# youmi-zym/TemporalStereo

Hardware: AMD Instinct MI355X
Metric: stereo pairs/sec, FlyingThings3D 540x960 D=192 (aggregation hot path) (higher is better)
Workload: dtype f32

## Files before the change

### temporalstereo_amd/csrc/conv_x6p.hip

```cpp
#include "conv_common.hpp"
#include "conv_x6p.hpp"

namespace {

typedef float f32x16 __attribute__((ext_vector_type(16)));
typedef __attribute__((address_space(3))) void* lds_ptr_t;

constexpr int XP_NC = 16;
constexpr int XP_WROWS = 3 * 9 * 2;
constexpr int XP_WBUF = XP_WROWS * 32;
constexpr int XP_GSLOTS = 10;
constexpr int XP_MAXC = 512;

__device__ __forceinline__ void phase_barrier() {
  asm volatile("s_waitcnt lgkmcnt(0)\n\ts_barrier" ::: "memory");
}

template <int HR>
struct XPG {
  static constexpr int in_rows = HR + 2, QPR = 10, LCOLS = 40, NPIX = in_rows * LCOLS;
  static constexpr int SLOTS = in_rows * QPR;
  static constexpr int NPB = HR / 4;
  static constexpr int HALF_U = 3 * 2 * NPIX;
  static constexpr int NWB = HR == 4 ? 3 : 2;
  static constexpr int SPC = HR == 4 ? 4 : 2;
  static constexpr int NCH = 16 / SPC;
  static constexpr int TILE0 = NWB * XP_WBUF;
  static constexpr size_t lds_bytes = (static_cast<size_t>(TILE0) + 2 * HALF_U) * 16 + (8 * 8 * (NPB * 32 + 4) + 2 * XP_MAXC) * 4;
  static_assert(SPC * SLOTS <= 256, "staging slots");
};

struct XPTile {
  int b, od, co0, ty0, tx0;
  int c0, c1;
  int ks;
};

template <int HR>
__global__ void __launch_bounds__(512, 2)
ig_conv_x6p_kernel(const float* __restrict__ x, const u32x4* __restrict__ w6, const float* __restrict__ scale,
                   const float* __restrict__ shift, float* __restrict__ y, const ts::X6P p) {
  using G = XPG<HR>;
  extern __shared__ __attribute__((aligned(16))) u32x4 ldsp[];
  constexpr int NPIX = G::NPIX, LCOLS = G::LCOLS, NPB = G::NPB;
  const int half = threadIdx.x >> 8, tid = threadIdx.x & 255;
  const int wave = tid >> 6, lane = tid & 63;
  const int px = lane & 31, grp = lane >> 5;
  u32x4* wls = ldsp;
  u32x4* in6 = ldsp + G::TILE0 + half * G::HALF_U;

  const int total = p.total_tiles;
  const int nwg = gridDim.x, g = blockIdx.x;
  int band0, band1, first, step;
  if (p.xcd && nwg % 8 == 0) {
    const int per = (total + 7) / 8, xcd = g & 7;
    band0 = xcd * per; band1 = min(total, band0 + per);
    first = band0 + (g >> 3); step = nwg >> 3;
  } else {
    band0 = 0; band1 = total; first = g; step = nwg;
  }
  const int nchunk = (p.Cin + XP_NC - 1) / XP_NC;
  auto tile_at = [&](int L) {
    XPTile t;
    const int tile = L % p.tiles_pp;
    int r = L / p.tiles_pp;
    const int cog = r % p.co_groups; r /= p.co_groups;
    t.od = r % p.D; r /= p.D;
    t.b = r % p.B; t.ks = r / p.B;
    t.c0 = t.ks * p.kspan; t.c1 = min(nchunk, t.c0 + p.kspan);
    t.co0 = cog * 32;
    t.ty0 = (tile / p.tiles_x) * (2 * HR) + half * HR;
    t.tx0 = (tile % p.tiles_x) * 32;
    return t;
  };
  const unsigned HW = static_cast<unsigned>(p.H) * p.W;
  const unsigned cstride_b = static_cast<unsigned>(p.in_cstride) * 4u;

  constexpr int SPC = G::SPC, NCH = G::NCH;
  const bool stager = tid < SPC * G::SLOTS;
  const int sg = SPC == 2 ? tid / G::SLOTS : tid / (2 * G::SLOTS);
  const int shalf = SPC == 2 ? 0 : (tid & 1);
  const int sslot = SPC == 2 ? tid - sg * G::SLOTS : (tid - sg * 2 * G::SLOTS) >> 1;
  const int srow = sslot / G::QPR, squad = sslot - srow * G::QPR;
  const int lpix = sg * NPIX + srow * LCOLS + 4 * squad;
  const int wsw = (sslot >> 1) & 1;
  const __amdgpu_buffer_rsrc_t wr = ig_rsrc(w6, p.w_bytes);
  const unsigned wchunk_b = static_cast<unsigned>(3 * XP_GSLOTS * 2 * p.coutp) * 16u;

  unsigned long long* trc = (p.trace && g == p.trace_wg && (tid == 0)) ? p.trace + half * 256 : nullptr;
  int ntr = 0;
  auto stamp = [&]() {
    if (trc && ntr < 250) trc[ntr] = __builtin_amdgcn_s_memtime();
    ++ntr;
  };
  stamp();
  unsigned long long* wgt = (p.trace && p.trace_wg == -2 && threadIdx.x == 0 && g < 8000) ? p.trace + 512 + 4 * g : nullptr;
  if (wgt) { wgt[0] = __builtin_amdgcn_s_memtime(); wgt[3] = __builtin_amdgcn_s_memrealtime(); }

  __amdgpu_buffer_rsrc_t xr;
  unsigned goff = kOOB;
  auto aim = [&](const XPTile& t) {
    xr = ig_rsrc(x + static_cast<long long>(t.b) * p.in_bstride, p.in_bytes);
    const int gy = t.ty0 - 1 + srow, gx = t.tx0 - 4 + 4 * squad;
    goff = (stager && gy >= 0 && gy < p.H && gx >= 0 && gx < p.W)
        ? (static_cast<unsigned>(t.od) * HW + static_cast<unsigned>(gy) * p.W + gx) * 4u : kOOB;
  };
  v4f rin[NCH];
  auto fetch = [&](int c) {
#pragma unroll
    for (int e = 0; e < NCH; ++e) {
      const unsigned co = static_cast<unsigned>(min(c * XP_NC + sg * 8 + shalf * 4 + e, p.Cin - 1)) * cstride_b;
      rin[e] = __builtin_bit_cast(v4f, __builtin_amdgcn_raw_buffer_load_b128(xr, (goff == kOOB || (p.dbg & 1)) ? kOOB : goff + co, 0, 0));
    }
  };
  auto dma_weights = [&](int c, int co0, int buf, int share) {
    u32x4* dst = wls + buf * XP_WBUF;
    const unsigned cbase = static_cast<unsigned>(c) * wchunk_b;
    const bool lane_ok = co0 + px < p.coutp && !(p.dbg & 16);
#pragma unroll
    for (int q = 0; q < 7; ++q) {
      const int i = share < 0 ? wave + 4 * q : 2 * (wave + 4 * q) + share;
      if (i < 27 && (share < 0 || q < 4)) {
        const int pt = i / 9, tap = i - pt * 9;
        const unsigned row = static_cast<unsigned>((pt * XP_GSLOTS + tap) * 2 + grp);
        const unsigned off = lane_ok ? (row * p.coutp + co0 + px) * 16u + cbase : kOOB;
        __builtin_amdgcn_raw_ptr_buffer_load_lds(wr, (lds_ptr_t)(dst + i * 64), 16, off, 0, 0, 0);
      }
    }
  };
  auto commit = [&]() {
    if (stager && !(p.dbg & 4)) {
#pragma unroll
      for (int i = 0; i < 4; ++i) {
        unsigned part[3][NCH / 2];
#pragma unroll
        for (int e = 0; e < NCH / 2; ++e) split6(rin[2 * e][i], rin[2 * e + 1][i], part[0][e], part[1][e], part[2][e]);
#pragma unroll
        for (int pt = 0; pt < 3; ++pt) {
          if constexpr (SPC == 2) in6[pt * 2 * NPIX + lpix + (i ^ wsw)] = u32x4{part[pt][0], part[pt][1], part[pt][2], part[pt][3]};
          else reinterpret_cast<u32x2*>(in6 + pt * 2 * NPIX + lpix + (i ^ wsw))[shalf] = u32x2{part[pt][0], part[pt][1]};
        }
      }
    }
  };

  auto swz = [](int P) { return (P & ~3) | ((P & 3) ^ ((P >> 3) & 1)); };
  int rbase[2][3];
#pragma unroll
  for (int rr = 0; rr < 2; ++rr)
#pragma unroll
    for (int kx = 0; kx < 3; ++kx) rbase[rr][kx] = grp * NPIX + swz((wave * NPB + rr) * LCOLS + 3 + kx + px);
  const int aoff = grp * 32 + px;

  constexpr int CH = NPB == 1 ? 2 : 1;
  constexpr int NACC = CH * NPB;
  f32x16 acc[NPB];

  constexpr int EPITCH = NPB * 32 + 4;
  float* scr = reinterpret_cast<float*>(ldsp + G::TILE0 + 2 * G::HALF_U) + (threadIdx.x >> 6) * (8 * EPITCH);
  const float* ss = reinterpret_cast<const float*>(ldsp + G::TILE0 + 2 * G::HALF_U) + 8 * 8 * EPITCH;
  auto epilogue = [&](const XPTile& t) {
    const bool split = p.ksplit > 1;
    const __amdgpu_buffer_rsrc_t yr = split
        ? ig_rsrc(p.partial + (static_cast<size_t>(t.ks) * p.B + t.b) * p.Cout * (static_cast<size_t>(p.D) * HW), p.part_bytes)
        : ig_rsrc(y + static_cast<long long>(t.b) * p.out_bstride, p.out_bytes);
    const unsigned ocs = split ? static_cast<unsigned>(p.D) * HW * 4u : static_cast<unsigned>(p.out_cstride) * 4u;
    const float* ab = (p.addend && !split) ? p.addend + static_cast<size_t>(t.b) * p.add_bstride : nullptr;
    const unsigned obase = static_cast<unsigned>(t.od) * HW;
    if (ab) {
#pragma unroll
      for (int r = 0; r < 16; ++r)
#pragma unroll
        for (int pb = 0; pb < NPB; ++pb) {
          const int oy = t.ty0 + wave * NPB + pb, ox = t.tx0 + px;
          acc[pb][r] += ab[static_cast<size_t>(min(t.co0 + (r & 3) + 8 * (r >> 2) + 4 * grp, p.Cout - 1)) * p.add_cstride +
                           ((oy < p.H && ox < p.W) ? static_cast<unsigned>(oy) * p.W + ox : 0u)];
        }
    }
#pragma unroll
    for (int r = 0; r < 16; ++r) {
      const int cc = min(t.co0 + (r & 3) + 8 * (r >> 2) + 4 * grp, p.coutp - 1);
      const float sc = split ? 1.f : ss[cc], sh = split ? 0.f : ss[XP_MAXC + cc];
#pragma unroll
      for (int pb = 0; pb < NPB; ++pb) acc[pb][r] = acc[pb][r] * sc + sh;
    }
    if (split) {
    } else if (p.act == ACT_SILU) {
#pragma unroll
      for (int r = 0; r < 16; ++r)
#pragma unroll
        for (int pb = 0; pb < NPB; ++pb) acc[pb][r] = silu_fast(acc[pb][r]);
    } else if (p.act == ACT_RELU) {
#pragma unroll
      for (int r = 0; r < 16; ++r)
#pragma unroll
        for (int pb = 0; pb < NPB; ++pb) acc[pb][r] = fmaxf(acc[pb][r], 0.f);
    }
#pragma unroll
    for (int k = 0; k < 4; ++k) {
#pragma unroll
      for (int j = 0; j < 4; ++j)
#pragma unroll
        for (int pb = 0; pb < NPB; ++pb) scr[(j + 4 * grp) * EPITCH + pb * 32 + px] = acc[pb][4 * k + j];
#pragma unroll
      for (int m = 0; m < NPB; ++m) {
        const int i = lane + 64 * m;
        const int c8 = i / (8 * NPB), q = i % (8 * NPB);
        const v4f val = *reinterpret_cast<const v4f*>(scr + c8 * EPITCH + q * 4);
        const int oy = t.ty0 + wave * NPB + (q >> 3), ox = t.tx0 + (q & 7) * 4;
        const int co = t.co0 + 8 * k + c8;
        const unsigned off = (oy < p.H && ox < p.W && co < p.Cout && !(p.dbg & 8))
            ? (obase + static_cast<unsigned>(oy) * p.W + ox) * 4u + static_cast<unsigned>(co) * ocs : kOOB;
        __builtin_amdgcn_raw_buffer_store_b128(__builtin_bit_cast(u32x4, val), yr, off, 0, 0);
      }
    }
  };

  if (first >= band1) return;
  {
    float* ssw = reinterpret_cast<float*>(ldsp + G::TILE0 + 2 * G::HALF_U) + 8 * 8 * EPITCH;
    for (int i = threadIdx.x; i < p.coutp; i += 512) {
      ssw[i] = scale ? scale[i] : 1.f;
      ssw[XP_MAXC + i] = shift ? shift[i] : 0.f;
    }
  }
  XPTile cur = tile_at(first);
  aim(cur);
  fetch(cur.c0);
  constexpr int NWB = G::NWB;
  if (NWB == 3) dma_weights(cur.c0, cur.co0, 0, half);
  else if (half == 1) dma_weights(cur.c0, cur.co0, 0, -1);
  if (half == 1) {
    asm volatile("s_waitcnt vmcnt(0)" ::: "memory");
    phase_barrier();
  }
  stamp();
  int wcur = 0, wnext = 1;
  for (int L = first; L < band1; L += step) {
    const bool more = L + step < band1;
    const XPTile nxt = more ? tile_at(L + step) : cur;
#pragma unroll
    for (int pb = 0; pb < NPB; ++pb)
#pragma unroll
      for (int r = 0; r < 16; ++r) acc[pb][r] = 0.f;
    for (int c = cur.c0; c < cur.c1; ++c, wcur = wnext, wnext = (wnext + 1 == NWB ? 0 : wnext + 1)) {
      const bool last = c + 1 == cur.c1;
      asm volatile("s_waitcnt vmcnt(0)" ::: "memory");
      stamp();
      if ((NWB == 3 || half == 1) && (!last || more))
        dma_weights(last ? nxt.c0 : c + 1, last ? nxt.co0 : cur.co0, wnext, NWB == 3 ? half : -1);
      commit();
      asm volatile("s_waitcnt lgkmcnt(0)" ::: "memory");
      stamp();
      phase_barrier();
      stamp();
      if (!last) fetch(c + 1);
      else if (more) { aim(nxt); fetch(nxt.c0); }
      const u32x4* wb = wls + wcur * XP_WBUF;
      f32x16 part[NACC];
#pragma unroll
      for (int a = 0; a < NACC; ++a)
#pragma unroll
        for (int r = 0; r < 16; ++r) part[a][r] = 0.f;
      bf16x8 af[2][3], bf[2][3][NPB];
      auto load_frag = [&](int tap, int buf) {
        constexpr int OA[3] = {0, 2, 1}, OB[3] = {2, 0, 1};
#pragma unroll
        for (int k = 0; k < 3; ++k) {
          af[buf][OA[k]] = __builtin_bit_cast(bf16x8, wb[(OA[k] * 9 + tap) * 64 + aoff]);
#pragma unroll
          for (int pb = 0; pb < NPB; ++pb) bf[buf][OB[k]][pb] = __builtin_bit_cast(bf16x8, in6[OB[k] * 2 * NPIX + rbase[(pb + tap / 3) & 1][tap % 3] + ((pb + tap / 3) >> 1) * 80]);
        }
      };
      if (!(p.dbg & 2)) {
        load_frag(0, 0);
        __builtin_amdgcn_sched_group_barrier(0x100, 3 + 3 * NPB, 0);
#pragma unroll
        for (int tap = 0; tap < 9; ++tap) {
          if (tap + 1 < 9) load_frag(tap + 1, (tap + 1) & 1);
          constexpr int PA[6] = {0, 2, 1, 0, 1, 0}, PB[6] = {2, 0, 1, 1, 0, 0};
#pragma unroll
          for (int t = 0; t < 6; ++t)
#pragma unroll
            for (int pb = 0; pb < NPB; ++pb) {
              const int a = pb * CH + (t % CH);
              part[a] = __builtin_amdgcn_mfma_f32_32x32x16_bf16(af[tap & 1][PA[t]], bf[tap & 1][PB[t]][pb], part[a], 0, 0, 0);
            }
          if (tap + 1 < 9) {
#pragma unroll
            for (int k = 0; k < 3 + 3 * NPB; ++k) {
              __builtin_amdgcn_sched_group_barrier(0x008, 1, 0);
              __builtin_amdgcn_sched_group_barrier(0x100, 1, 0);
            }
            if constexpr (6 * NPB > 3 + 3 * NPB) __builtin_amdgcn_sched_group_barrier(0x008, 6 * NPB - (3 + 3 * NPB), 0);
          } else {
            __builtin_amdgcn_sched_group_barrier(0x008, 6 * NPB, 0);
          }
        }
      }
#pragma unroll
      for (int pb = 0; pb < NPB; ++pb)
#pragma unroll
        for (int r = 0; r < 16; ++r) {
          float v = part[pb * CH][r];
#pragma unroll
          for (int k = 1; k < CH; ++k) v += part[pb * CH + k][r];
          acc[pb][r] += v;
        }
      if (trc) asm volatile("s_nop 0" :: "v"(acc[0][0]), "v"(acc[NPB - 1][15]));
      stamp();
      if (NWB == 3 || half == 1) asm volatile("s_waitcnt vmcnt(%0)" :: "n"(NCH) : "memory");
      phase_barrier();
      stamp();
    }
    epilogue(cur);
    stamp();
    cur = nxt;
  }
  if (wgt) { asm volatile("s_waitcnt vmcnt(0)" ::: "memory"); wgt[1] = __builtin_amdgcn_s_memtime(); wgt[2] = __builtin_amdgcn_s_memrealtime(); }
  if (half == 0) phase_barrier();
}

template <int HR>
int launch_x6p(const float* x, const void* w6, const float* scale, const float* shift, float* y, const ts::X6P& p, int nwg, hipStream_t st) {
  constexpr size_t lds = XPG<HR>::lds_bytes;
  static_assert(lds <= 160 * 1024, "ig_conv_x6p_kernel: LDS");
  auto kern = &ig_conv_x6p_kernel<HR>;
  static const int attr = hipFuncSetAttribute(reinterpret_cast<const void*>(kern), hipFuncAttributeMaxDynamicSharedMemorySize, static_cast<int>(lds));
  (void)attr;
  hipLaunchKernelGGL(kern, dim3(nwg), dim3(512), lds, st, x, static_cast<const u32x4*>(w6), scale, shift, y, p);
  return ts::launched("ig_conv_x6p_kernel");
}

}

namespace ts {

static unsigned long long* trace_buf = nullptr;
constexpr size_t kTraceBytes = 4096 + 8000 * 32;

static long long tiles_of(const X6P& p, int hr) {
  return static_cast<long long>((p.H + 2 * hr - 1) / (2 * hr)) * ((p.W + 31) / 32) * p.D * p.B * ((p.Cout + 31) / 32) * (p.ksplit > 1 ? p.ksplit : 1);
}

int x6p_rows(const X6P& p) {
  static const long long forced = env_ll("TS_X6P_HR", 0);
  if (forced == 4 || forced == 8) return static_cast<int>(forced);
  const long long r8 = (tiles_of(p, 8) + kNumCU - 1) / kNumCU, r4 = (tiles_of(p, 4) + kNumCU - 1) / kNumCU;
  return 100 * r8 <= 58 * r4 ? 8 : 4;
}

long long x6p_grid(const X6P& p) { return tiles_of(p, 4); }

int x6p_launch(const float* x, const void* w6, const float* scale, const float* shift, float* y, X6P p, void* stream) {
  const int hr = x6p_rows(p);
  static const long long dbg = env_ll("TS_X6P_DBG", 0);
  p.dbg = static_cast<int>(dbg);
  static const long long trace_wg = env_ll("TS_X6P_TRACE", -1);
  if (trace_wg != -1 && !trace_buf) { (void)hipMalloc(reinterpret_cast<void**>(&trace_buf), kTraceBytes); (void)hipMemset(trace_buf, 0, kTraceBytes); }
  p.trace = trace_buf; p.trace_wg = static_cast<int>(trace_wg);
  p.tiles_x = (p.W + 31) / 32;
  p.co_groups = (p.Cout + 31) / 32;
  p.tiles_pp = ((p.H + 2 * hr - 1) / (2 * hr)) * p.tiles_x;
  if (p.ksplit < 1) p.ksplit = 1;
  const long long total = static_cast<long long>(p.tiles_pp) * p.co_groups * p.D * p.B * p.ksplit;
  if (total > 0x3fffffff) return fail(TS_ERR_UNSUPPORTED, "conv3d_hw_x6: too many tiles");
  p.total_tiles = static_cast<int>(total);
  static const long long max_wgs0 = env_ll("TS_X6P_WGS", 208);
  static const long long splitk_all = env_ll("TS_X6P_SPLITK_ALL", 1);
  const long long max_wgs = (splitk_all && p.ksplit > 1 && total <= 256) ? 256 : max_wgs0;
  int nwg = static_cast<int>(total < max_wgs ? total : max_wgs);
  {
    const long long rounds = (total + nwg - 1) / nwg;
    const long long even = (total + rounds - 1) / rounds;
    nwg = static_cast<int>(((even + 7) / 8 * 8 <= nwg) ? (even + 7) / 8 * 8 : even);
  }
  hipStream_t st = as_stream(stream);
  return hr == 8 ? launch_x6p<8>(x, w6, scale, shift, y, p, nwg, st) : launch_x6p<4>(x, w6, scale, shift, y, p, nwg, st);
}

}

extern "C" int ts_x6p_trace_read(unsigned long long* host) {
  if (!ts::trace_buf) return -1;
  (void)hipDeviceSynchronize();
  return static_cast<int>(hipMemcpy(host, ts::trace_buf, ts::kTraceBytes, hipMemcpyDeviceToHost));
}
```

### temporalstereo_amd/csrc/conv_x6s.hip

```cpp
#include "conv_common.hpp"

namespace {

enum { XS_S2 = 0, XS_T3 = 1, XS_T4 = 2 };

template <int MODE, int TR = 8>
struct XG {
  static constexpr bool T = MODE != XS_S2;
  static constexpr int in_rows = T ? TR + 2 : 9;
  static constexpr int QPR = T ? 10 : 18;
  static constexpr int LCOLS = 4 * QPR;
  static constexpr int NPIX = in_rows * LCOLS, NPIXP = NPIX + 1;
  static constexpr int SLOTS = in_rows * QPR;
  static constexpr int NSLOT = T ? 16 : 12;
  static constexpr int NU = T ? 4 : 3;
  static constexpr int NPB = T ? TR / 2 : 2;
  static constexpr int EPI = T ? TR * 64 + 4 : 132;
};
constexpr int kEpiS2 = 132;

inline int slot_tap(int mode, int s) {
  if (mode == XS_S2) return s < 9 ? s : -1;
  const int ks = mode == XS_T4 ? 4 : 3;
  const int cls = s >> 2, a = (s >> 1) & 1, b = s & 1, pa = cls >> 1, pb = cls & 1;
  auto k = [&](int par, int opt) { return par ? (opt ? 0 : 2) : (opt ? (ks == 4 ? 3 : -1) : 1); };
  const int ky = k(pa, a), kx = k(pb, b);
  return (ky < 0 || kx < 0) ? -1 : ky * ks + kx;
}

struct SlotMap { int tap[16]; };

__global__ void __launch_bounds__(256)
weight_split6_g8_kernel(const float* __restrict__ w_t, u32x4* __restrict__ w6, int Cin, int ntaps, int wpad, int coutp, int nchunk,
                        int nslot, const SlotMap m) {
  const int n = nchunk * nslot * coutp;
  for (int i = blockIdx.x * blockDim.x + threadIdx.x; i < n; i += gridDim.x * blockDim.x) {
    const int co = i % coutp;
    const int r = i / coutp;
    const int slot = r % nslot, chunk = r / nslot;
    const int tap = m.tap[slot];
    float v[8];
#pragma unroll
    for (int e = 0; e < 8; ++e) {
      const int ci = chunk * 8 + e;
      v[e] = (tap >= 0 && ci < Cin && co < wpad) ? w_t[(static_cast<size_t>(ci) * ntaps + tap) * wpad + co] : 0.f;
    }
    unsigned part[3][4];
#pragma unroll
    for (int e = 0; e < 4; ++e) split6(v[2 * e], v[2 * e + 1], part[0][e], part[1][e], part[2][e]);
#pragma unroll
    for (int pt = 0; pt < 3; ++pt)
      w6[((static_cast<size_t>(chunk) * 3 + pt) * nslot + slot) * coutp + co] = u32x4{part[pt][0], part[pt][1], part[pt][2], part[pt][3]};
  }
}

template <int MODE, int CB, int TR = 8>
__global__ void __launch_bounds__(256, TR == 4 ? 3 : 2)
ig_conv_x6s_kernel(const float* __restrict__ x, const u32x4* __restrict__ w6, const float* __restrict__ scale,
                   const float* __restrict__ shift, float* __restrict__ y, const IG p) {
  extern __shared__ __attribute__((aligned(16))) u32x4 lds6[];
  using G = XG<MODE, TR>;
  constexpr bool T = G::T;
  static_assert(!T || CB == 1, "transposed forms: 16 output channels per workgroup (four classes of accumulators)");
  constexpr int LCOLS = G::LCOLS, NPIXP = G::NPIXP, NSLOT = G::NSLOT, NU = G::NU, NPB = G::NPB, SLOTS = G::SLOTS;
  constexpr int COB = CB * 16;
  constexpr int WV = 3 * NSLOT * COB, RWN = (WV + 255) / 256;
  constexpr int NCH = T ? 4 : 8;
  u32x4* in6 = lds6;
  u32x4* w6s = lds6 + 3 * NPIXP;

  const int wave = threadIdx.x >> 6, lane = threadIdx.x & 63;
  const int j = lane & 15, kq = lane >> 4;
  unsigned lin = blockIdx.x + gridDim.x * (blockIdx.y + gridDim.y * blockIdx.z);
  {
    const unsigned total = gridDim.x * gridDim.y * gridDim.z, per = total / 8;
    if (p.xcd && lin < per * 8) lin = (lin % 8) * per + lin / 8;
  }
  const int tile = lin % gridDim.x;
  const int od = (lin / gridDim.x) % gridDim.y;
  const int bz = lin / (gridDim.x * gridDim.y);
  const int cog = bz % p.co_groups, b = bz / p.co_groups;
  const int co0 = cog * COB;
  const int ty0 = (tile / p.tiles_x) * (T ? TR : 4), tx0 = (tile % p.tiles_x) * 32;
  const int row0 = T ? ty0 - 1 : 2 * ty0 - 1, col0 = T ? tx0 - 4 : 2 * tx0 - 4;
  const unsigned HW = static_cast<unsigned>(p.H) * p.W;
  const unsigned cstride_b = static_cast<unsigned>(p.in_cstride) * 4u;

  const int half = T ? static_cast<int>(threadIdx.x >> 7) : 0;
  const int sslot = T ? static_cast<int>(threadIdx.x & 127) : static_cast<int>(threadIdx.x);
  const bool stager = sslot < SLOTS;
  const int srow = sslot / G::QPR, squad = sslot - srow * G::QPR;
  unsigned goff = kOOB;
  {
    const int gy = row0 + srow, gx = col0 + 4 * squad;
    if (stager && gy >= 0 && gy < p.H && gx >= 0 && gx < p.W)
      goff = (static_cast<unsigned>(od) * HW + static_cast<unsigned>(gy) * p.W + gx) * 4u;
  }
  const int lpix = srow * LCOLS + 4 * squad;

  unsigned woff[RWN];
  int wl[RWN];
#pragma unroll
  for (int q = 0; q < RWN; ++q) {
    const int v = threadIdx.x + 256 * q;
    const int col = v % COB, r = v / COB;
    const bool ok = v < WV && co0 + col < p.coutp;
    woff[q] = ok ? static_cast<unsigned>(r * p.coutp + co0 + col) * 16u : kOOB;
    wl[q] = v < WV ? v : WV;
  }
  const __amdgpu_buffer_rsrc_t xr = ig_rsrc(x + static_cast<long long>(b) * p.in_bstride, p.in_bytes);
  const __amdgpu_buffer_rsrc_t wr = ig_rsrc(w6, p.w_bytes);
  const unsigned wchunk_b = static_cast<unsigned>(3 * NSLOT * p.coutp) * 16u;

  int boff[NPB], toff[NU];
#pragma unroll
  for (int pb = 0; pb < NPB; ++pb) {
    if (T) boff[pb] = ((TR == 8 ? wave * 2 + (pb >> 1) : wave) + 1) * LCOLS + 4 + (pb & 1) * 16 + j;
    else boff[pb] = (2 * wave) * LCOLS + 3 + 2 * (pb * 16 + j);
  }
#pragma unroll
  for (int u = 0; u < NU; ++u) {
    if (T) {
      const int pa = u >> 1, pbit = u & 1, a = kq >> 1, bq = kq & 1;
      const int dy = a ? (pa ? 1 : (MODE == XS_T4 ? -1 : 0)) : 0, dx = bq ? (pbit ? 1 : (MODE == XS_T4 ? -1 : 0)) : 0;
      toff[u] = dy * LCOLS + dx;
    } else {
      const int s = 4 * u + kq;
      toff[u] = s < 9 ? (s / 3) * LCOLS + (s % 3) : 0;
    }
  }
  const int aoff = kq * COB + j;

  v4f acc[T ? 4 : 1][CB][NPB];
#pragma unroll
  for (int c = 0; c < (T ? 4 : 1); ++c)
#pragma unroll
    for (int cb = 0; cb < CB; ++cb)
#pragma unroll
      for (int pb = 0; pb < NPB; ++pb) acc[c][cb][pb] = v4f{0.f, 0.f, 0.f, 0.f};
  float esc[CB][4], esh[CB][4];
#pragma unroll
  for (int cb = 0; cb < CB; ++cb)
#pragma unroll
    for (int r = 0; r < 4; ++r) {
      const int co = min(co0 + cb * 16 + kq * 4 + r, p.Cout - 1);
      esc[cb][r] = scale ? scale[co] : 1.f;
      esh[cb][r] = shift ? shift[co] : 0.f;
    }

  v4f rin[NCH];
  u32x4 rw[RWN];
  auto fetch = [&](int c0) {
#pragma unroll
    for (int c = 0; c < NCH; ++c) {
      const unsigned co = static_cast<unsigned>(min(c0 + half * 4 + c, p.Cin - 1)) * cstride_b;
      rin[c] = __builtin_bit_cast(v4f, __builtin_amdgcn_raw_buffer_load_b128(xr, goff == kOOB ? kOOB : goff + co, 0, 0));
    }
    const unsigned wso = static_cast<unsigned>(c0 / 8) * wchunk_b;
#pragma unroll
    for (int q = 0; q < RWN; ++q) rw[q] = __builtin_amdgcn_raw_buffer_load_b128(wr, woff[q], wso, 0);
  };
  auto commit = [&]() {
    if (stager) {
#pragma unroll
      for (int i = 0; i < 4; ++i) {
        unsigned part[3][NCH / 2];
#pragma unroll
        for (int e = 0; e < NCH / 2; ++e) split6(rin[2 * e][i], rin[2 * e + 1][i], part[0][e], part[1][e], part[2][e]);
#pragma unroll
        for (int pt = 0; pt < 3; ++pt) {
          if constexpr (T) reinterpret_cast<u32x2*>(in6 + pt * NPIXP + lpix + i)[half] = u32x2{part[pt][0], part[pt][1]};
          else in6[pt * NPIXP + lpix + i] = u32x4{part[pt][0], part[pt][1], part[pt][2], part[pt][3]};
        }
      }
    }
#pragma unroll
    for (int q = 0; q < RWN; ++q) w6s[wl[q]] = rw[q];
  };

  fetch(0);
  for (int c0 = 0; c0 < p.Cin; c0 += 8) {
    __syncthreads();
    commit();
    __syncthreads();
    if (c0 + 8 < p.Cin) fetch(c0 + 8);
    v4f part[CB][NPB];
    auto zero_part = [&]() {
#pragma unroll
      for (int cb = 0; cb < CB; ++cb)
#pragma unroll
        for (int pb = 0; pb < NPB; ++pb) part[cb][pb] = v4f{0.f, 0.f, 0.f, 0.f};
    };
    zero_part();
    bf16x8 a[2][3][CB], bv[2][3][NPB];
    auto load_frag = [&](int u, int buf) {
#pragma unroll
      for (int pt = 0; pt < 3; ++pt) {
#pragma unroll
        for (int cb = 0; cb < CB; ++cb) a[buf][pt][cb] = __builtin_bit_cast(bf16x8, w6s[(pt * NSLOT + 4 * u) * COB + aoff + cb * 16]);
#pragma unroll
        for (int pb = 0; pb < NPB; ++pb) bv[buf][pt][pb] = __builtin_bit_cast(bf16x8, in6[pt * NPIXP + boff[pb] + toff[u]]);
      }
    };
    load_frag(0, 0);
#pragma unroll
    for (int u = 0; u < NU; ++u) {
      if (u + 1 < NU) load_frag(u + 1, (u + 1) & 1);
      constexpr int PA[6] = {0, 2, 1, 0, 1, 0}, PB[6] = {2, 0, 1, 1, 0, 0};
#pragma unroll
      for (int t = 0; t < 6; ++t)
#pragma unroll
        for (int cb = 0; cb < CB; ++cb)
#pragma unroll
          for (int pb = 0; pb < NPB; ++pb)
            part[cb][pb] = __builtin_amdgcn_mfma_f32_16x16x32_bf16(a[u & 1][PA[t]][cb], bv[u & 1][PB[t]][pb], part[cb][pb], 0, 0, 0);
      if (T) {
#pragma unroll
        for (int cb = 0; cb < CB; ++cb)
#pragma unroll
          for (int pb = 0; pb < NPB; ++pb) acc[u][cb][pb] += part[cb][pb];
        zero_part();
      }
    }
    if (!T) {
#pragma unroll
      for (int cb = 0; cb < CB; ++cb)
#pragma unroll
        for (int pb = 0; pb < NPB; ++pb) acc[0][cb][pb] += part[cb][pb];
    }
  }

  const unsigned hw_o = static_cast<unsigned>(p.Ho) * p.Wo;
  const __amdgpu_buffer_rsrc_t yr = ig_rsrc(y + static_cast<long long>(b) * p.out_bstride, p.out_bytes);
  const unsigned ocs = static_cast<unsigned>(p.out_cstride) * 4u;
  const unsigned obase = static_cast<unsigned>(od) * hw_o;
  float* epi = reinterpret_cast<float*>(lds6);
  if constexpr (!T) {
    __syncthreads();
#pragma unroll
    for (int cb = 0; cb < CB; ++cb)
#pragma unroll
      for (int pb = 0; pb < NPB; ++pb)
#pragma unroll
        for (int r = 0; r < 4; ++r) {
          const int co = co0 + cb * 16 + kq * 4 + r;
          epi[(cb * 16 + kq * 4 + r) * kEpiS2 + wave * 32 + pb * 16 + j] =
              apply_act(acc[0][cb][pb][r] * esc[cb][r] + esh[cb][r], p.act, p.act_param, co);
        }
    __syncthreads();
#pragma unroll
    for (int it = 0; it < CB * 2; ++it) {
      const int idx = static_cast<int>(threadIdx.x) + 256 * it;
      const int col = idx >> 5, q = idx & 31;
      const int oy = ty0 + (q >> 3), ox = tx0 + (q & 7) * 4;
      const u32x4 val = *reinterpret_cast<const u32x4*>(epi + col * kEpiS2 + q * 4);
      const int co = co0 + col;
      const unsigned off = (oy < p.Ho && ox < p.Wo && co < p.Cout)
          ? (obase + static_cast<unsigned>(oy) * p.Wo + ox) * 4u + static_cast<unsigned>(co) * ocs : kOOB;
      __builtin_amdgcn_raw_buffer_store_b128(val, yr, off, 0, 0);
    }
  } else {
#pragma unroll
    for (int pa = 0; pa < 2; ++pa) {
      __syncthreads();
#pragma unroll
      for (int pbit = 0; pbit < 2; ++pbit)
#pragma unroll
        for (int pb = 0; pb < NPB; ++pb)
#pragma unroll
          for (int r = 0; r < 4; ++r) {
            const int co = co0 + kq * 4 + r;
            epi[(kq * 4 + r) * G::EPI + (TR == 8 ? wave * 2 + (pb >> 1) : wave) * 64 + 2 * ((pb & 1) * 16 + j) + pbit] =
                apply_act(acc[pa * 2 + pbit][0][pb][r] * esc[0][r] + esh[0][r], p.act, p.act_param, co);
          }
      __syncthreads();
#pragma unroll
      for (int it = 0; it < TR; ++it) {
        const int idx = static_cast<int>(threadIdx.x) + 256 * it;
        const int col = idx / (TR * 16), rem = idx % (TR * 16);
        const int row = rem >> 4, q = rem & 15;
        const int iy = ty0 + row, oy = 2 * iy + pa, ox = 2 * tx0 + 4 * q;
        const u32x4 val = *reinterpret_cast<const u32x4*>(epi + col * G::EPI + row * 64 + q * 4);
        const int co = co0 + col;
        const unsigned off = (iy < p.H && oy < p.Ho && ox < p.Wo && co < p.Cout)
            ? (obase + static_cast<unsigned>(oy) * p.Wo + ox) * 4u + static_cast<unsigned>(co) * ocs : kOOB;
        __builtin_amdgcn_raw_buffer_store_b128(val, yr, off, 0, 0);
      }
    }
  }
}

template <int MODE, int CB, int TR = 8>
int launch_x6s(const float* x, const void* w6, const float* scale, const float* shift, float* y, const IG& p, dim3 grid, hipStream_t st) {
  using G = XG<MODE, TR>;
  constexpr size_t main_b = (static_cast<size_t>(3) * G::NPIXP + 3 * G::NSLOT * CB * 16 + 1) * 16;
  constexpr size_t epi_b = G::T ? static_cast<size_t>(16) * G::EPI * 4 : static_cast<size_t>(CB) * 16 * kEpiS2 * 4;
  constexpr size_t lds = main_b > epi_b ? main_b : epi_b;
  static_assert(lds <= 64 * 1024, "ig_conv_x6s_kernel: LDS tile");
  hipLaunchKernelGGL((ig_conv_x6s_kernel<MODE, CB, TR>), grid, dim3(256), lds, st, x, static_cast<const u32x4*>(w6), scale, shift, y, p);
  return ts::launched("ig_conv_x6s_kernel");
}

inline int coutp6(int Cout) { return (Cout + 15) / 16 * 16; }
inline int mode_taps(int mode) { return mode == XS_T4 ? 16 : 9; }
inline int mode_slots(int mode) { return mode == XS_S2 ? 12 : 16; }
}

extern "C" int ts_conv3d_hw_x6s_supported(int Cin, int Cout, int H, int W, int mode) {
  if (mode < 0 || mode > 2 || Cin < 16 || Cout <= 0 || Cout > 512 || H <= 0 || W <= 0 || W % 4) return 0;
  if (mode == XS_S2) return (((W - 1) / 2 + 1) % 4) == 0;
  return 1;
}

extern "C" size_t ts_conv3d_hw_x6s_weight_bytes(int Cin, int Cout, int mode) {
  if (Cin <= 0 || Cout <= 0 || Cout > 512 || mode < 0 || mode > 2) return 0;
  return static_cast<size_t>((Cin + 7) / 8) * 3 * mode_slots(mode) * coutp6(Cout) * 16;
}

extern "C" int ts_conv3d_hw_x6s_weight_split(const float* w_t, void* w6, int Cin, int Cout, int w_pad, int mode, void* stream) {
  TS_REQUIRE(Cin > 0 && Cout > 0 && Cout <= 512 && w_pad >= Cout, TS_ERR_SHAPE, "conv3d_hw_x6s_weight_split: bad channel counts");
  TS_REQUIRE(mode >= 0 && mode <= 2, TS_ERR_SHAPE, "conv3d_hw_x6s_weight_split: unknown mode %d", mode);
  TS_REQUIRE_PTR(w_t); TS_REQUIRE_PTR(w6);
  const int nchunk = (Cin + 7) / 8, nslot = mode_slots(mode), cp = coutp6(Cout);
  SlotMap m;
  for (int s = 0; s < 16; ++s) m.tap[s] = s < nslot ? slot_tap(mode, s) : -1;
  const int n = nchunk * nslot * cp;
  hipLaunchKernelGGL(weight_split6_g8_kernel, dim3((n + 255) / 256), dim3(256), 0, ts::as_stream(stream), w_t,
                     static_cast<u32x4*>(w6), Cin, mode_taps(mode), w_pad, cp, nchunk, nslot, m);
  return ts::launched("weight_split6_g8_kernel");
}

extern "C" int ts_conv3d_hw_x6s_fwd(const float* x, const void* w6, const float* scale, const float* shift, float* y,
                                    int B, int Cin, int Cout, int D, int H, int W, int mode, int act, float act_param,
                                    long long in_bstride, long long in_cstride, long long out_bstride, long long out_cstride,
                                    void* stream) {
  TS_REQUIRE(B > 0 && Cin > 0 && Cout > 0 && D > 0 && H > 0 && W > 0, TS_ERR_SHAPE, "conv3d_hw_x6s: non-positive size");
  TS_REQUIRE(ts_conv3d_hw_x6s_supported(Cin, Cout, H, W, mode), TS_ERR_UNSUPPORTED,
             "conv3d_hw_x6s: needs Cin >= 16, Cout <= 512, W %% 4 == 0 and Wo %% 4 == 0 (Cin=%d Cout=%d W=%d mode=%d)", Cin, Cout, W, mode);
  TS_REQUIRE(act >= 0 && act <= 4, TS_ERR_SHAPE, "conv3d_hw_x6s: unknown activation");
  TS_REQUIRE(D <= 65535, TS_ERR_UNSUPPORTED, "conv3d_hw_x6s: grid too large");
  TS_REQUIRE_PTR(x); TS_REQUIRE_PTR(w6); TS_REQUIRE_PTR(y);
  IG p;
  p.Cin = Cin; p.Cout = Cout; p.coutp = coutp6(Cout); p.D = D; p.H = H; p.W = W; p.Do = D;
  if (mode == XS_S2) { p.Ho = (H - 1) / 2 + 1; p.Wo = (W - 1) / 2 + 1; }
  else { p.Ho = 2 * H; p.Wo = 2 * W; }
  p.stride = 2; p.dil = 1; p.pad = 1; p.k = mode == XS_T4 ? 4 : 3; p.transposed = mode != XS_S2;
  p.act = act; p.act_param = act_param;
  p.in_bstride = in_bstride; p.in_cstride = in_cstride; p.out_bstride = out_bstride; p.out_cstride = out_cstride;
  p.ksplit = 1; p.kspan = Cin; p.partial = nullptr; p.B = B; p.part_bytes = 0;
  p.addend = nullptr; p.add_bstride = p.add_cstride = p.add_dstride = 0;
  static const int xcd = env_not_zero("TS_X6_XCD") ? 1 : 0;
  p.xcd = xcd;
  {
    const unsigned long long in_b = (static_cast<unsigned long long>(Cin - 1) * in_cstride + static_cast<unsigned long long>(D) * H * W) * 4ull;
    const unsigned long long out_b = (static_cast<unsigned long long>(Cout - 1) * out_cstride + static_cast<unsigned long long>(D) * p.Ho * p.Wo) * 4ull;
    const unsigned long long w_b = ts_conv3d_hw_x6s_weight_bytes(Cin, Cout, mode);
    TS_REQUIRE(in_b < 0x7fffffffull && out_b < 0x7fffffffull && w_b < 0x7fffffffull && in_cstride >= 0 && out_cstride >= 0,
               TS_ERR_UNSUPPORTED, "conv3d_hw_x6s: a batch element spans 2 GiB or more");
    p.in_bytes = static_cast<unsigned>(in_b); p.out_bytes = static_cast<unsigned>(out_b); p.w_bytes = static_cast<unsigned>(w_b);
  }
  hipStream_t st = ts::as_stream(stream);
  TS_REQUIRE(static_cast<long long>(B) * ((p.coutp + 15) / 16) <= 65535, TS_ERR_UNSUPPORTED, "conv3d_hw_x6s: batch x channel groups beyond the grid's z extent");
  if (mode == XS_S2) {
    p.tiles_x = (p.Wo + 31) / 32;
    const int tiles = ((p.Ho + 3) / 4) * p.tiles_x;
    const int cb = Cout > 16 ? 2 : 1;
    p.co_groups = (p.coutp / 16 + cb - 1) / cb;
    const dim3 grid(tiles, D, B * p.co_groups);
    return cb == 2 ? launch_x6s<XS_S2, 2>(x, w6, scale, shift, y, p, grid, st) : launch_x6s<XS_S2, 1>(x, w6, scale, shift, y, p, grid, st);
  }
  p.tiles_x = (W + 31) / 32;
  p.co_groups = p.coutp / 16;
  static const long long tr_env = env_ll("TS_X6S_TR", 0);
  const long long wgs8 = static_cast<long long>((H + 7) / 8) * p.tiles_x * D * B * p.co_groups;
  const long long tr = tr_env ? tr_env : (wgs8 < 3 * ts::kNumCU / 2 ? 4 : 8);
  if (tr == 4) {
    const dim3 grid(((H + 3) / 4) * p.tiles_x, D, B * p.co_groups);
    return mode == XS_T4 ? launch_x6s<XS_T4, 1, 4>(x, w6, scale, shift, y, p, grid, st) : launch_x6s<XS_T3, 1, 4>(x, w6, scale, shift, y, p, grid, st);
  }
  const int tiles = ((H + 7) / 8) * p.tiles_x;
  const dim3 grid(tiles, D, B * p.co_groups);
  return mode == XS_T4 ? launch_x6s<XS_T4, 1>(x, w6, scale, shift, y, p, grid, st) : launch_x6s<XS_T3, 1>(x, w6, scale, shift, y, p, grid, st);
}
```

Measured before the change: 1495.

## Add persistent pipelined stride-2 conv kernel and compile out x6p debug hooks

Adds a persistent, double-half 512-thread kernel for the stride-2 hw conv that keeps weights in triple-buffered LDS via buffer-to-LDS DMA, prefetches input chunks for the next tile, and walks tiles with an XCD-aware schedule. It is gated behind the TS_X6SP environment variable, so the default path is unchanged. Separately, the x6p kernel's debug and trace branches are compiled out unless TS_X6P_INSTRUMENT is defined, removing runtime dbg checks and trace pointer logic from the hot loop.

```diff
diff --git a/temporalstereo_amd/csrc/conv_x6p.hip b/temporalstereo_amd/csrc/conv_x6p.hip
--- a/temporalstereo_amd/csrc/conv_x6p.hip
+++ b/temporalstereo_amd/csrc/conv_x6p.hip
@@ -11,6 +11,12 @@
 constexpr int XP_WBUF = XP_WROWS * 32;
 constexpr int XP_GSLOTS = 10;
 constexpr int XP_MAXC = 512;
+
+#ifdef TS_X6P_INSTRUMENT
+#define XP_DBG(bit) (p.dbg & (bit))
+#else
+#define XP_DBG(bit) 0
+#endif
 
 __device__ __forceinline__ void phase_barrier() {
   asm volatile("s_waitcnt lgkmcnt(0)\n\ts_barrier" ::: "memory");
@@ -87,6 +93,7 @@
   const __amdgpu_buffer_rsrc_t wr = ig_rsrc(w6, p.w_bytes);
   const unsigned wchunk_b = static_cast<unsigned>(3 * XP_GSLOTS * 2 * p.coutp) * 16u;
 
+#ifdef TS_X6P_INSTRUMENT
   unsigned long long* trc = (p.trace && g == p.trace_wg && (tid == 0)) ? p.trace + half * 256 : nullptr;
   int ntr = 0;
   auto stamp = [&]() {
@@ -96,6 +103,9 @@
   stamp();
   unsigned long long* wgt = (p.trace && p.trace_wg == -2 && threadIdx.x == 0 && g < 8000) ? p.trace + 512 + 4 * g : nullptr;
   if (wgt) { wgt[0] = __builtin_amdgcn_s_memtime(); wgt[3] = __builtin_amdgcn_s_memrealtime(); }
+#else
+  auto stamp = []() {};
+#endif
 
   __amdgpu_buffer_rsrc_t xr;
   unsigned goff = kOOB;
@@ -110,13 +120,13 @@
 #pragma unroll
     for (int e = 0; e < NCH; ++e) {
       const unsigned co = static_cast<unsigned>(min(c * XP_NC + sg * 8 + shalf * 4 + e, p.Cin - 1)) * cstride_b;
-      rin[e] = __builtin_bit_cast(v4f, __builtin_amdgcn_raw_buffer_load_b128(xr, (goff == kOOB || (p.dbg & 1)) ? kOOB : goff + co, 0, 0));
+      rin[e] = __builtin_bit_cast(v4f, __builtin_amdgcn_raw_buffer_load_b128(xr, (goff == kOOB || XP_DBG(1)) ? kOOB : goff + co, 0, 0));
     }
   };
   auto dma_weights = [&](int c, int co0, int buf, int share) {
     u32x4* dst = wls + buf * XP_WBUF;
     const unsigned cbase = static_cast<unsigned>(c) * wchunk_b;
-    const bool lane_ok = co0 + px < p.coutp && !(p.dbg & 16);
+    const bool lane_ok = co0 + px < p.coutp && !XP_DBG(16);
 #pragma unroll
     for (int q = 0; q < 7; ++q) {
       const int i = share < 0 ? wave + 4 * q : 2 * (wave + 4 * q) + share;
@@ -129,7 +139,7 @@
     }
   };
   auto commit = [&]() {
-    if (stager && !(p.dbg & 4)) {
+    if (stager && !XP_DBG(4)) {
 #pragma unroll
       for (int i = 0; i < 4; ++i) {
         unsigned part[3][NCH / 2];
@@ -209,7 +219,7 @@
         const v4f val = *reinterpret_cast<const v4f*>(scr + c8 * EPITCH + q * 4);
         const int oy = t.ty0 + wave * NPB + (q >> 3), ox = t.tx0 + (q & 7) * 4;
         const int co = t.co0 + 8 * k + c8;
-        const unsigned off = (oy < p.H && ox < p.W && co < p.Cout && !(p.dbg & 8))
+        const unsigned off = (oy < p.H && ox < p.W && co < p.Cout && !XP_DBG(8))
             ? (obase + static_cast<unsigned>(oy) * p.W + ox) * 4u + static_cast<unsigned>(co) * ocs : kOOB;
         __builtin_amdgcn_raw_buffer_store_b128(__builtin_bit_cast(u32x4, val), yr, off, 0, 0);
       }
@@ -272,7 +282,7 @@
           for (int pb = 0; pb < NPB; ++pb) bf[buf][OB[k]][pb] = __builtin_bit_cast(bf16x8, in6[OB[k] * 2 * NPIX + rbase[(pb + tap / 3) & 1][tap % 3] + ((pb + tap / 3) >> 1) * 80]);
         }
       };
-      if (!(p.dbg & 2)) {
+      if (!XP_DBG(2)) {
         load_frag(0, 0);
         __builtin_amdgcn_sched_group_barrier(0x100, 3 + 3 * NPB, 0);
 #pragma unroll
@@ -307,7 +317,9 @@
           for (int k = 1; k < CH; ++k) v += part[pb * CH + k][r];
           acc[pb][r] += v;
         }
+#ifdef TS_X6P_INSTRUMENT
       if (trc) asm volatile("s_nop 0" :: "v"(acc[0][0]), "v"(acc[NPB - 1][15]));
+#endif
       stamp();
       if (NWB == 3 || half == 1) asm volatile("s_waitcnt vmcnt(%0)" :: "n"(NCH) : "memory");
       phase_barrier();
@@ -317,7 +329,9 @@
     stamp();
     cur = nxt;
   }
+#ifdef TS_X6P_INSTRUMENT
   if (wgt) { asm volatile("s_waitcnt vmcnt(0)" ::: "memory"); wgt[1] = __builtin_amdgcn_s_memtime(); wgt[2] = __builtin_amdgcn_s_memrealtime(); }
+#endif
   if (half == 0) phase_barrier();
 }
 
@@ -354,11 +368,15 @@
 
 int x6p_launch(const float* x, const void* w6, const float* scale, const float* shift, float* y, X6P p, void* stream) {
   const int hr = x6p_rows(p);
+#ifdef TS_X6P_INSTRUMENT
   static const long long dbg = env_ll("TS_X6P_DBG", 0);
   p.dbg = static_cast<int>(dbg);
   static const long long trace_wg = env_ll("TS_X6P_TRACE", -1);
   if (trace_wg != -1 && !trace_buf) { (void)hipMalloc(reinterpret_cast<void**>(&trace_buf), kTraceBytes); (void)hipMemset(trace_buf, 0, kTraceBytes); }
   p.trace = trace_buf; p.trace_wg = static_cast<int>(trace_wg);
+#else
+  p.dbg = 0; p.trace = nullptr; p.trace_wg = -1;
+#endif
   p.tiles_x = (p.W + 31) / 32;
   p.co_groups = (p.Cout + 31) / 32;
   p.tiles_pp = ((p.H + 2 * hr - 1) / (2 * hr)) * p.tiles_x;
diff --git a/temporalstereo_amd/csrc/conv_x6s.hip b/temporalstereo_amd/csrc/conv_x6s.hip
--- a/temporalstereo_amd/csrc/conv_x6s.hip
+++ b/temporalstereo_amd/csrc/conv_x6s.hip
@@ -290,6 +290,240 @@
   }
 }
 
+namespace sp {
+constexpr int ROWS = 9, QPR = 17, RUN = 34, RU = 2 * RUN;
+constexpr int PART = ROWS * RU;
+constexpr int HALF_U = 3 * PART;
+constexpr int SLOTS = ROWS * QPR;
+constexpr int NSLOT = 12, NU = 5;
+constexpr int WBUF = 3 * 2 * NU * 32;
+constexpr int NWB = 3;
+constexpr int TILE0 = NWB * WBUF;
+constexpr int EPITCH = 36;
+constexpr int MAXC = 512;
+constexpr size_t lds_bytes = (static_cast<size_t>(TILE0) + 2 * HALF_U) * 16 + (8 * 8 * EPITCH + 2 * MAXC) * 4;
+static_assert(TILE0 * 16 <= 65536, "LDS-DMA destinations inside the first 64 KB");
+static_assert(SLOTS <= 256, "staging slots");
+}
+
+struct XSP {
+  int Cin, Cout, coutp, B, D, H, W, Ho, Wo;
+  int act;
+  float act_param;
+  long long in_bstride, in_cstride, out_bstride, out_cstride;
+  unsigned in_bytes, w_bytes, out_bytes;
+  int xcd;
+  int tiles_x, co_groups, tiles_pp, total_tiles;
+};
+
+__device__ __forceinline__ void sp_phase_barrier() {
+  asm volatile("s_waitcnt lgkmcnt(0)\n\ts_barrier" ::: "memory");
+}
+
+__global__ void __launch_bounds__(512, 2)
+ig_conv_x6sp_kernel(const float* __restrict__ x, const u32x4* __restrict__ w6, const float* __restrict__ scale,
+                    const float* __restrict__ shift, float* __restrict__ y, const XSP p) {
+  typedef float f32x16 __attribute__((ext_vector_type(16)));
+  typedef __attribute__((address_space(3))) void* lds_ptr_t;
+  using namespace sp;
+  extern __shared__ __attribute__((aligned(16))) u32x4 ldsp[];
+  const int half = threadIdx.x >> 8, tid = threadIdx.x & 255;
+  const int wave = tid >> 6, lane = tid & 63;
+  const int px = lane & 31, grp = lane >> 5;
+  u32x4* wls = ldsp;
+  u32x4* in6 = ldsp + TILE0 + half * HALF_U;
+
+  const int total = p.total_tiles;
+  const int nwg = gridDim.x, g = blockIdx.x;
+  int band1, first, step;
+  if (p.xcd && nwg % 8 == 0) {
+    const int per = (total + 7) / 8, xcd = g & 7;
+    band1 = min(total, xcd * per + per);
+    first = xcd * per + (g >> 3); step = nwg >> 3;
+  } else {
+    band1 = total; first = g; step = nwg;
+  }
+  if (first >= band1) return;
+  const int nchunk = (p.Cin + 7) / 8;
+  struct Tile { int b, od, co0, ty0, tx0; };
+  auto tile_at = [&](int L) {
+    Tile t;
+    const int tile = L % p.tiles_pp;
+    int r = L / p.tiles_pp;
+    const int cog = r % p.co_groups; r /= p.co_groups;
+    t.od = r % p.D; t.b = r / p.D;
+    t.co0 = cog * 32;
+    t.ty0 = (tile / p.tiles_x) * 8 + half * 4;
+    t.tx0 = (tile % p.tiles_x) * 32;
+    return t;
+  };
+  const unsigned HW = static_cast<unsigned>(p.H) * p.W;
+  const unsigned cstride_b = static_cast<unsigned>(p.in_cstride) * 4u;
+
+  const bool stager = tid < SLOTS;
+  const int srow = tid / QPR, squad = tid - srow * QPR;
+  const int lunit = srow * RU + 2 * squad;
+  const __amdgpu_buffer_rsrc_t wr = ig_rsrc(w6, p.w_bytes);
+  const unsigned wchunk_b = static_cast<unsigned>(3 * NSLOT * p.coutp) * 16u;
+
+  __amdgpu_buffer_rsrc_t xr;
+  unsigned goff = kOOB;
+  auto aim = [&](const Tile& t) {
+    xr = ig_rsrc(x + static_cast<long long>(t.b) * p.in_bstride, p.in_bytes);
+    const int gy = 2 * t.ty0 - 1 + srow, gx = 2 * t.tx0 - 4 + 4 * squad;
+    goff = (stager && gy >= 0 && gy < p.H && gx >= 0 && gx < p.W)
+        ? (static_cast<unsigned>(t.od) * HW + static_cast<unsigned>(gy) * p.W + gx) * 4u : kOOB;
+  };
+  v4f rin[8];
+  auto fetch = [&](int c) {
+#pragma unroll
+    for (int e = 0; e < 8; ++e) {
+      const unsigned co = static_cast<unsigned>(min(c * 8 + e, p.Cin - 1)) * cstride_b;
+      rin[e] = __builtin_bit_cast(v4f, __builtin_amdgcn_raw_buffer_load_b128(xr, goff == kOOB ? kOOB : goff + co, 0, 0));
+    }
+  };
+  auto dma_weights = [&](int c, int co0, int buf) {
+    u32x4* dst = wls + buf * WBUF;
+    const unsigned cbase = static_cast<unsigned>(c) * wchunk_b;
+    const bool lane_ok = co0 + px < p.coutp;
+#pragma unroll
+    for (int q = 0; q < 2; ++q) {
+      const int i = 2 * (wave + 4 * q) + half;
+      if (i < 3 * NU) {
+        const int pt = i / NU, u = i - pt * NU;
+        const unsigned row = static_cast<unsigned>(pt * NSLOT + 2 * u + grp);
+        const unsigned off = lane_ok ? (row * p.coutp + co0 + px) * 16u + cbase : kOOB;
+        __builtin_amdgcn_raw_ptr_buffer_load_lds(wr, (lds_ptr_t)(dst + i * 64), 16, off, 0, 0, 0);
+      }
+    }
+  };
+  auto commit = [&]() {
+    if (stager) {
+#pragma unroll
+      for (int i = 0; i < 4; ++i) {
+        unsigned part[3][4];
+#pragma unroll
+        for (int e = 0; e < 4; ++e) split6(rin[2 * e][i], rin[2 * e + 1][i], part[0][e], part[1][e], part[2][e]);
+#pragma unroll
+        for (int pt = 0; pt < 3; ++pt) in6[pt * PART + lunit + (i & 1) * RUN + (i >> 1)] = u32x4{part[pt][0], part[pt][1], part[pt][2], part[pt][3]};
+      }
+    }
+  };
+
+  int boff[NU];
+#pragma unroll
+  for (int u = 0; u < NU; ++u) {
+    const int s = min(2 * u + grp, 8), ky = s / 3, kx = s - 3 * ky;
+    boff[u] = (2 * wave + ky) * RU + (kx == 1 ? 0 : RUN) + px + (kx == 0 ? 1 : 2);
+  }
+  const int aoff = grp * 32 + px;
+
+  f32x16 acc;
+  float* scr = reinterpret_cast<float*>(ldsp + TILE0 + 2 * HALF_U) + (threadIdx.x >> 6) * (8 * EPITCH);
+  const float* ss = reinterpret_cast<const float*>(ldsp + TILE0 + 2 * HALF_U) + 8 * 8 * EPITCH;
+  auto epilogue = [&](const Tile& t) {
+    const __amdgpu_buffer_rsrc_t yr = ig_rsrc(y + static_cast<long long>(t.b) * p.out_bstride, p.out_bytes);
+    const unsigned ocs = static_cast<unsigned>(p.out_cstride) * 4u;
+    const unsigned obase = static_cast<unsigned>(t.od) * (static_cast<unsigned>(p.Ho) * p.Wo);
+#pragma unroll
+    for (int r = 0; r < 16; ++r) {
+      const int cc = min(t.co0 + (r & 3) + 8 * (r >> 2) + 4 * grp, p.coutp - 1);
+      acc[r] = acc[r] * ss[cc] + ss[MAXC + cc];
+    }
+    if (p.act == ACT_SILU) {
+#pragma unroll
+      for (int r = 0; r < 16; ++r) acc[r] = silu_fast(acc[r]);
+    } else if (p.act != ACT_NONE) {
+#pragma unroll
+      for (int r = 0; r < 16; ++r) acc[r] = apply_act(acc[r], p.act, p.act_param, t.co0 + (r & 3) + 8 * (r >> 2) + 4 * grp);
+    }
+#pragma unroll
+    for (int k = 0; k < 4; ++k) {
+#pragma unroll
+      for (int j = 0; j < 4; ++j) scr[(j + 4 * grp) * EPITCH + px] = acc[4 * k + j];
+      const int c8 = lane >> 3, q = lane & 7;
+      const v4f val = *reinterpret_cast<const v4f*>(scr + c8 * EPITCH + q * 4);
+      const int oy = t.ty0 + wave, ox = t.tx0 + q * 4;
+      const int co = t.co0 + 8 * k + c8;
+      const unsigned off = (oy < p.Ho && ox < p.Wo && co < p.Cout)
+          ? (obase + static_cast<unsigned>(oy) * p.Wo + ox) * 4u + static_cast<unsigned>(co) * ocs : kOOB;
+      __builtin_amdgcn_raw_buffer_store_b128(__builtin_bit_cast(u32x4, val), yr, off, 0, 0);
+    }
+  };
+
+  {
+    float* ssw = reinterpret_cast<float*>(ldsp + TILE0 + 2 * HALF_U) + 8 * 8 * EPITCH;
+    for (int i = threadIdx.x; i < p.coutp; i += 512) {
+      ssw[i] = scale ? scale[i] : 1.f;
+      ssw[MAXC + i] = shift ? shift[i] : 0.f;
+    }
+  }
+  Tile cur = tile_at(first);
+  aim(cur);
+  fetch(0);
+  dma_weights(0, cur.co0, 0);
+  if (half == 1) {
+    asm volatile("s_waitcnt vmcnt(0)" ::: "memory");
+    sp_phase_barrier();
+  }
+  int wcur = 0, wnext = 1;
+  for (int L = first; L < band1; L += step) {
+    const bool more = L + step < band1;
+    const Tile nxt = more ? tile_at(L + step) : cur;
+#pragma unroll
+    for (int r = 0; r < 16; ++r) acc[r] = 0.f;
+    for (int c = 0; c < nchunk; ++c, wcur = wnext, wnext = (wnext + 1 == NWB ? 0 : wnext + 1)) {
+      const bool last = c + 1 == nchunk;
+      asm volatile("s_waitcnt vmcnt(0)" ::: "memory");
+      if (!last || more) dma_weights(last ? 0 : c + 1, last ? nxt.co0 : cur.co0, wnext);
+      commit();
+      sp_phase_barrier();
+      if (!last) fetch(c + 1);
+      else if (more) { aim(nxt); fetch(0); }
+      const u32x4* wb = wls + wcur * WBUF;
+      f32x16 part[2];
+#pragma unroll
+      for (int a = 0; a < 2; ++a)
+#pragma unroll
+        for (int r = 0; r < 16; ++r) part[a][r] = 0.f;
+      bf16x8 af[2][3], bf[2][3];
+      auto load_frag = [&](int u, int buf) {
+        constexpr int OA[3] = {0, 2, 1}, OB[3] = {2, 0, 1};
+#pragma unroll
+        for (int k = 0; k < 3; ++k) {
+          af[buf][OA[k]] = __builtin_bit_cast(bf16x8, wb[(OA[k] * NU + u) * 64 + aoff]);
+          bf[buf][OB[k]] = __builtin_bit_cast(bf16x8, in6[OB[k] * PART + boff[u]]);
+        }
+      };
+      load_frag(0, 0);
+      __builtin_amdgcn_sched_group_barrier(0x100, 6, 0);
+#pragma unroll
+      for (int u = 0; u < NU; ++u) {
+        if (u + 1 < NU) load_frag(u + 1, (u + 1) & 1);
+        constexpr int PA[6] = {0, 2, 1, 0, 1, 0}, PB[6] = {2, 0, 1, 1, 0, 0};
+#pragma unroll
+        for (int t = 0; t < 6; ++t) part[t & 1] = __builtin_amdgcn_mfma_f32_32x32x16_bf16(af[u & 1][PA[t]], bf[u & 1][PB[t]], part[t & 1], 0, 0, 0);
+        if (u + 1 < NU) {
+#pragma unroll
+          for (int k = 0; k < 6; ++k) {
+            __builtin_amdgcn_sched_group_barrier(0x008, 1, 0);
+            __builtin_amdgcn_sched_group_barrier(0x100, 1, 0);
+          }
+        } else {
+          __builtin_amdgcn_sched_group_barrier(0x008, 6, 0);
+        }
+      }
+#pragma unroll
+      for (int r = 0; r < 16; ++r) acc[r] += part[0][r] + part[1][r];
+      asm volatile("s_waitcnt vmcnt(8)" ::: "memory");
+      sp_phase_barrier();
+    }
+    epilogue(cur);
+    cur = nxt;
+  }
+  if (half == 0) sp_phase_barrier();
+}
+
 template <int MODE, int CB, int TR = 8>
 int launch_x6s(const float* x, const void* w6, const float* scale, const float* shift, float* y, const IG& p, dim3 grid, hipStream_t st) {
   using G = XG<MODE, TR>;
@@ -299,6 +533,29 @@
   static_assert(lds <= 64 * 1024, "ig_conv_x6s_kernel: LDS tile");
   hipLaunchKernelGGL((ig_conv_x6s_kernel<MODE, CB, TR>), grid, dim3(256), lds, st, x, static_cast<const u32x4*>(w6), scale, shift, y, p);
   return ts::launched("ig_conv_x6s_kernel");
+}
+
+int launch_x6sp(const float* x, const void* w6, const float* scale, const float* shift, float* y, XSP q, hipStream_t st) {
+  q.tiles_x = (q.Wo + 31) / 32;
+  q.co_groups = (q.Cout + 31) / 32;
+  q.tiles_pp = ((q.Ho + 7) / 8) * q.tiles_x;
+  const long long total = static_cast<long long>(q.tiles_pp) * q.co_groups * q.D * q.B;
+  if (total > 0x3fffffff) return ts::fail(TS_ERR_UNSUPPORTED, "conv3d_hw_x6s: too many tiles");
+  q.total_tiles = static_cast<int>(total);
+  static const long long max_wgs = env_ll("TS_X6SP_WGS", 208);
+  int nwg = static_cast<int>(total < max_wgs ? total : max_wgs);
+  {
+    const long long rounds = (total + nwg - 1) / nwg;
+    const long long even = (total + rounds - 1) / rounds;
+    nwg = static_cast<int>(((even + 7) / 8 * 8 <= nwg) ? (even + 7) / 8 * 8 : even);
+  }
+  constexpr size_t lds = sp::lds_bytes;
+  static_assert(lds <= 160 * 1024, "ig_conv_x6sp_kernel: LDS");
+  static const int attr = hipFuncSetAttribute(reinterpret_cast<const void*>(&ig_conv_x6sp_kernel), hipFuncAttributeMaxDynamicSharedMemorySize,
+                                              static_cast<int>(lds));
+  (void)attr;
+  hipLaunchKernelGGL(ig_conv_x6sp_kernel, dim3(nwg), dim3(512), lds, st, x, static_cast<const u32x4*>(w6), scale, shift, y, q);
+  return ts::launched("ig_conv_x6sp_kernel");
 }
 
 inline int coutp6(int Cout) { return (Cout + 15) / 16 * 16; }
@@ -361,6 +618,15 @@
   }
   hipStream_t st = ts::as_stream(stream);
   TS_REQUIRE(static_cast<long long>(B) * ((p.coutp + 15) / 16) <= 65535, TS_ERR_UNSUPPORTED, "conv3d_hw_x6s: batch x channel groups beyond the grid's z extent");
+  static const bool sp_on = env_not_zero("TS_X6SP");
+  if (mode == XS_S2 && sp_on) {
+    XSP q;
+    q.Cin = Cin; q.Cout = Cout; q.coutp = p.coutp; q.B = B; q.D = D; q.H = H; q.W = W; q.Ho = p.Ho; q.Wo = p.Wo;
+    q.act = act; q.act_param = act_param;
+    q.in_bstride = in_bstride; q.in_cstride = in_cstride; q.out_bstride = out_bstride; q.out_cstride = out_cstride;
+    q.in_bytes = p.in_bytes; q.w_bytes = p.w_bytes; q.out_bytes = p.out_bytes; q.xcd = p.xcd;
+    return launch_x6sp(x, w6, scale, shift, y, q, st);
+  }
   if (mode == XS_S2) {
     p.tiles_x = (p.Wo + 31) / 32;
     const int tiles = ((p.Ho + 3) / 4) * p.tiles_x;
```

Measured after the change: 1508, median of 6. Within noise of the previous version (+0.9%).
